# jeongminpark417/COALA-GNN

Hardware: AMD Instinct MI355X
Metric: feature-gather GB/s (payload = rows x dim x 4 B delivered per second), IGB-medium GraphSAGE minibatch fetch (higher is better)
Workload: dtype f32

## Files before the change

coala-gnn_amd/csrc/coala_cache.hip:

```cpp
#include <hip/hip_runtime.h>
#include <hip/hip_ext.h>

#include <algorithm>
#include <cstdarg>
#include <cstdio>
#include <cstdlib>
#include <cstring>
#include <new>
#include <type_traits>
#include <utility>
#include <vector>

#include "../../include/coala_hip.h"
#include "coala_internal.h"

namespace {

constexpr uint64_t kEmptyKey = 0xFFFFFFFFFFFFFFFFull;
constexpr uint32_t kLinkMiss = 0x80000000u;
constexpr uint32_t kLinkBad = 0x7FFFFFFFu;
constexpr int kStatBlocks = 2048;
constexpr int kFillSlots = 8;

struct CacheDev {
    void* keys;
    uint64_t* set_cnt;
    uint32_t* color_meta;
    int32_t* color_counters;
    const int32_t* node_color;
    float* lines;
    const float* cold;
    uint64_t num_sets;
    uint64_t num_rows;
    uint32_t cache_dim;
    uint32_t dim;
    uint32_t n_gpus;
    int32_t gshift;
    int32_t sshift;
    uint32_t distributed;
    uint32_t cold_partitioned;
    uint32_t tag32;
    uint64_t* set_head;
    uint32_t* miss_link;
    unsigned long long* stats;
};

__device__ __forceinline__ uint64_t set_of(const CacheDev& c, uint64_t id) {
    uint64_t k = id;
    if (c.distributed) {
        if (c.gshift >= 0) k = id >> c.gshift;
        else if ((id >> 32) == 0) k = (uint32_t)id / c.n_gpus;
        else k = id / c.n_gpus;
    }
    if (c.sshift >= 0) return k & (c.num_sets - 1);
    if ((k >> 32) == 0 && (c.num_sets >> 32) == 0) return (uint32_t)k % (uint32_t)c.num_sets;
    return k % c.num_sets;
}

__device__ __forceinline__ uint64_t cold_row_of(const CacheDev& c, uint64_t id) {
    if (!c.cold_partitioned) return id;
    if (c.gshift >= 0) return id >> c.gshift;
    return id / c.n_gpus;
}

constexpr int kMaxRanges = 64;
struct RangeSet {
// ... 62 lines not shown

constexpr int kK1MinWaves = 4;
constexpr int kK1Passes = 4;
constexpr int64_t kK1SingleMaxChunks = 1 << 20;
constexpr int kK1Waves = 2;
#ifdef COALA_DEV_KNOBS
constexpr int kK1MaxWaves = 4;
#else
constexpr int kK1MaxWaves = kK1Waves;
#endif

template <typename V> __device__ __forceinline__ V nt_load(const V* p) { return __builtin_nontemporal_load(p); }
template <typename V> __device__ __forceinline__ void nt_store(V v, V* p) { __builtin_nontemporal_store(v, p); }

template <int CD, int VEC, typename TAG, int NP, bool FULL, bool REDIR, bool SINGLE>
__global__ __launch_bounds__(64 * kK1MaxWaves, kK1MinWaves) void probe_gather_kernel(const int64_t* __restrict__ idx, float* __restrict__ out,
                                                                    int64_t n, uint32_t gen, uint32_t n_blocks, CacheDev c, Redirect rd) {
    using G = Geo<CD, VEC, NP>;
    using V = typename VecT<VEC>::type;
    using TG = TagGeo<TAG>;
    using TV = typename TG::vec;
    constexpr int R = G::R;
    static_assert(R <= 32, "per-chunk row masks are 32 bits wide");
    if (blockIdx.x == 0 && threadIdx.x < kFillSlots) reinterpret_cast<uint32_t*>(c.stats + 2 * kStatBlocks)[(gen & 1u) * kFillSlots + threadIdx.x] = 0u;
    uint32_t* fill_flag = reinterpret_cast<uint32_t*>(c.stats + 2 * kStatBlocks) + 2 * kFillSlots;
    if (blockIdx.x == 0 && threadIdx.x == kFillSlots) fill_flag[(gen + 1u) & 1u] = 0u;
    constexpr int TSTEPS = (R + TG::SPL - 1) / TG::SPL;
    int lane = threadIdx.x & 63;
#ifdef COALA_DEV_KNOBS
    const int wpb = (int)(blockDim.x >> 6);
#else
    constexpr int wpb = kK1Waves;
#endif
    const int64_t wave = (int64_t)blockIdx.x * wpb + (threadIdx.x >> 6);
    const int64_t n_waves = (int64_t)n_blocks * wpb;
    const int64_t n_chunks = (n + R - 1) / R;
    const uint32_t nunits = c.dim / VEC;
    const TAG* __restrict__ keys = reinterpret_cast<const TAG*>(c.keys);

    struct Ids { uint64_t id[TSTEPS]; bool valid[TSTEPS]; int32_t drow[REDIR ? TSTEPS : 1]; };
    struct Tags { uint64_t id[TSTEPS]; uint32_t set[TSTEPS]; TV kk[TSTEPS]; bool ok[TSTEPS]; bool valid[TSTEPS]; int32_t drow[REDIR ? TSTEPS : 1]; };
    auto load_ids = [&](int64_t chunk) {
        Ids r;
#pragma unroll
        for (int t = 0; t < TSTEPS; ++t) {
            const int q_l = t * TG::SPL + lane / TG::LPS;
            const int64_t i_l = chunk * R + q_l;
// ... 110 lines not shown
            }
#pragma unroll
            for (int v = 0; v < G::VPL; ++v) {
                const uint32_t u = v * G::LPR + l_in;
                if (FULL || u < nunits) {
                    if (h) dst[u] = val[p][v];
                    else if (bad) dst[u] = V(0.0f);
                }
            }
        }
#pragma unroll
        for (int t = 0; t < TSTEPS; ++t) {
            if (lead_l[t]) {
                uint32_t w = 0u;
                if (imiss_l[t]) w = kLinkMiss | (((uint32_t)(prev[t] >> 32) == gen) ? (uint32_t)prev[t] : 0u);
                else if (bad_l[t]) w = kLinkBad;
                c.miss_link[base + t * TG::SPL + lane / TG::LPS] = w;
            }
        }
        if (SINGLE) break;
    }
}

__device__ __forceinline__ uint64_t shfl64(uint64_t v, int src) {
    const uint32_t lo = __shfl((int)(uint32_t)v, src), hi = __shfl((int)(uint32_t)(v >> 32), src);
    return ((uint64_t)hi << 32) | lo;
}

template <int CD, int VEC, bool REDIR = false, int NP = 4>
__global__ __launch_bounds__(256) void miss_fill_kernel(CacheDev c, const int64_t* __restrict__ idx, float* __restrict__ out,
                                                        int tile_rows, int sparse_max, uint32_t gen, RangeSet rs, Redirect rd, int dyn_slot) {
    using G = Geo<CD, VEC, NP>;
    using V = typename VecT<VEC>::type;
    constexpr int R = G::R;
    const int lane = threadIdx.x & 63;
    const int64_t wave = (int64_t)blockIdx.x * (blockDim.x >> 6) + (threadIdx.x >> 6);
    const int64_t n_waves = (int64_t)gridDim.x * (blockDim.x >> 6);
    const int64_t n_tiles = ((int64_t)rs.total + tile_rows - 1) / tile_rows;
    const int chunks_per_tile = tile_rows / R;
    const uint32_t nunits = c.dim / VEC;
    const int sub = (G::RPP == 2) ? (lane >> 5) : 0;
    const int l_in = lane & (G::LPR - 1);
    uint32_t my_miss = 0, my_bad = 0;

    constexpr int U = 8;
    uint32_t* ticket = reinterpret_cast<uint32_t*>(c.stats + 2 * kStatBlocks) + (dyn_slot < 0 ? 0 : dyn_slot);
    const bool dyn = dyn_slot >= 0;
    if (reinterpret_cast<const uint32_t*>(c.stats + 2 * kStatBlocks)[2 * kFillSlots + (gen & 1u)] == 0u) return;
    const int64_t n_deal = dyn ? 1 : n_waves;
    const int64_t even8 = n_tiles / (n_waves * 8);
    const int claim_min = even8 < 1 ? 1 : (even8 > U ? U : (int)even8);
    int claim = claim_min;
    for (int64_t unit = dyn ? -1 : wave;;) {
      int64_t claim_end = n_tiles;
      if (dyn) {
          uint32_t t = 0;
          if (lane == 0) t = atomicAdd(ticket, (uint32_t)claim);
          unit = (int64_t)(uint32_t)__builtin_amdgcn_readfirstlane((int)t);
          if (unit >= n_tiles) break;
          claim_end = unit + claim < n_tiles ? unit + claim : n_tiles;
          claim = claim * 2 > 4 * U ? 4 * U : claim * 2;
      } else if (unit >= n_tiles) break;
     for (int64_t tile0 = unit; tile0 < claim_end; tile0 += n_deal * U) {
      const int n_here = dyn ? (int)(claim_end - tile0 < U ? claim_end - tile0 : U) : U;
      uint64_t st_pack = 0;
#pragma unroll
      for (int u = 0; u < U; ++u) {
          const int64_t tile = tile0 + u * n_deal;
          const uint32_t p = (u < n_here && tile < n_tiles && lane < tile_rows) ? pos_of(rs, (uint32_t)(tile * tile_rows + lane)) : 0xFFFFFFFFu;
          const uint32_t w = (p != 0xFFFFFFFFu) ? c.miss_link[p] : 0u;
          const uint64_t v = (w == 0u) ? 0u : ((w & kLinkMiss) ? 1u : 2u);
          st_pack |= v << (8 * u);
      }
      if (!__ballot(st_pack != 0)) continue;
      uint32_t slot_l = 0, win_l = 0;
      uint64_t id_l = 0;
      int64_t drow_l = 0;
      auto rank_at = [&](uint32_t pos) {
          id_l = (uint64_t)idx[pos];
          drow_l = (int64_t)pos;
          if (REDIR && (int64_t)pos >= rd.begin && (int64_t)pos < rd.end)
              drow_l = -((rd.row_map ? rd.row_map[(int64_t)pos - rd.begin] : (int64_t)pos - rd.begin) + 1);
          const uint64_t set = set_of(c, id_l);
          uint32_t cur = (uint32_t)c.set_head[set];
          uint32_t total = 0, rank = 0;
          while (cur) {
              const uint32_t p2 = cur - 1;
              ++total;
              rank += (p2 < pos) ? 1u : 0u;
              cur = c.miss_link[p2] & ~kLinkMiss;
          }
          const uint64_t cv = __hip_atomic_load(c.set_cnt + set, __ATOMIC_RELAXED, __HIP_MEMORY_SCOPE_AGENT);
          const uint32_t cnt0 = ((uint32_t)(cv >> 32) == gen) ? (uint32_t)cv - total : (uint32_t)cv;
          if (rank == 0) __hip_atomic_store(c.set_cnt + set, ((uint64_t)gen << 32) | (uint32_t)(cnt0 + total), __ATOMIC_RELAXED, __HIP_MEMORY_SCOPE_AGENT);
          const uint32_t way = (cnt0 + rank) & (COALA_WAYS - 1);
          slot_l = (uint32_t)(set * COALA_WAYS) + way;
          win_l = (rank + COALA_WAYS >= total) ? 1u : 0u;
          if (win_l) {
              if (c.tag32) reinterpret_cast<uint32_t*>(c.keys)[slot_l] = (uint32_t)id_l;
              else reinterpret_cast<uint64_t*>(c.keys)[slot_l] = id_l;
              if (c.color_counters) {
                  const int32_t col = c.node_color[id_l];
                  atomicSub(c.color_counters + c.color_meta[slot_l], 1);
                  atomicAdd(c.color_counters + col, 1);
                  c.color_meta[slot_l] = (uint32_t)col;
              }
          }
      };
      auto move_group = [&](const int (&srcl)[G::PASSES], const bool (&live)[G::PASSES]) {
          V val[G::PASSES][G::VPL];
          uint32_t slot_[G::PASSES];
          uint64_t id[G::PASSES];
          int64_t drow[G::PASSES];
          bool winner[G::PASSES];
#pragma unroll
          for (int p = 0; p < G::PASSES; ++p) {
              slot_[p] = (uint32_t)__shfl((int)slot_l, srcl[p]);
              winner[p] = __shfl((int)win_l, srcl[p]) != 0;
              id[p] = shfl64(id_l, srcl[p]);
              drow[p] = (int64_t)shfl64((uint64_t)drow_l, srcl[p]);
          }
#pragma unroll
          for (int p = 0; p < G::PASSES; ++p) {
              const V* src = reinterpret_cast<const V*>(c.cold + cold_row_of(c, id[p]) * (uint64_t)c.dim);
#pragma unroll
              for (int v = 0; v < G::VPL; ++v) {
                  const uint32_t u = v * G::LPR + l_in;
                  if (live[p] && u < nunits) val[p][v] = nt_load(src + u);
              }
          }
#pragma unroll
          for (int p = 0; p < G::PASSES; ++p) {
              V* dst = (REDIR && drow[p] < 0) ? reinterpret_cast<V*>(rd.out + (uint64_t)(-(drow[p] + 1)) * c.dim)
                                              : reinterpret_cast<V*>(out + (uint64_t)drow[p] * c.dim);
              V* line = reinterpret_cast<V*>(c.lines + (uint64_t)slot_[p] * CD);
#pragma unroll
              for (int v = 0; v < G::VPL; ++v) {
                  const uint32_t u = v * G::LPR + l_in;
                  if (live[p] && u < nunits) {
                      nt_store(val[p][v], dst + u);
                      if (winner[p]) nt_store(val[p][v], line + u);
                  }
              }
          }
      };
      auto stream_holders = [&](uint64_t holders) {
          int srcl[G::PASSES];
          bool live[G::PASSES];
          while (holders) {
#pragma unroll
              for (int p = 0; p < G::PASSES; ++p) {
                  int l0 = -1, l1 = -1;
                  if (holders) { l0 = __builtin_ctzll(holders); holders &= holders - 1; }
                  if (G::RPP == 2 && holders) { l1 = __builtin_ctzll(holders); holders &= holders - 1; }
                  const int l = (G::RPP == 2 && sub) ? l1 : l0;
                  live[p] = l >= 0;
                  srcl[p] = l >= 0 ? l : 0;
              }
              move_group(srcl, live);
          }
      };
      uint64_t mmask[U];
      uint32_t total_miss = 0, worst = 0;
#pragma unroll
      for (int u = 0; u < U; ++u) {
          const uint8_t st = (uint8_t)(st_pack >> (8 * u));
          mmask[u] = __ballot(st == 1);
          my_miss += (st == 1);
          my_bad += (st == 2);
          const uint32_t cnt = (uint32_t)__builtin_popcountll(mmask[u]);
          total_miss += cnt;
          worst = cnt > worst ? cnt : worst;
      }
      if (!total_miss) continue;
      claim = claim_min;
      if (total_miss <= 64 && (int)worst <= sparse_max) {
          uint32_t k = (uint32_t)lane;
          int u_sel = -1;
          uint64_t m_sel = 0;
#pragma unroll
          for (int u = 0; u < U; ++u) {
              const uint32_t cnt = (uint32_t)__builtin_popcountll(mmask[u]);
              if (u_sel < 0) {
                  if (k < cnt) { u_sel = u; m_sel = mmask[u]; }
                  else k -= cnt;
              }
          }
          if (u_sel >= 0) {
              for (uint32_t i = 0; i < k; ++i) m_sel &= m_sel - 1;
              const uint32_t pos = pos_of(rs, (uint32_t)((tile0 + u_sel * n_deal) * tile_rows + __builtin_ctzll(m_sel)));
              rank_at(pos);
          }
          stream_holders(total_miss >= 64 ? ~0ull : ((1ull << total_miss) - 1ull));
          continue;
      }
#pragma nounroll
      for (int u = 0; u < U; ++u) {
        const uint8_t st = (uint8_t)(st_pack >> (8 * u));
        const uint64_t tile_mask = __ballot(st == 1);
        if (!tile_mask) continue;
        const uint32_t pos_l = st ? pos_of(rs, (uint32_t)((tile0 + u * n_deal) * tile_rows + lane)) : 0u;
        if (__builtin_popcountll(tile_mask) <= sparse_max) {
            if (st == 1) rank_at(pos_l);
            stream_holders(tile_mask);
        } else {
            int srcl[G::PASSES];
            bool live[G::PASSES];
            for (int ck = 0; ck < chunks_per_tile; ++ck) {
                const uint32_t live_mask = (uint32_t)(tile_mask >> (ck * R)) & ((1u << R) - 1u);
                if (!live_mask) continue;
                const int lane0 = ck * R;
                if (st == 1 && lane >= lane0 && lane < lane0 + R) rank_at(pos_l);
#pragma unroll
                for (int p = 0; p < G::PASSES; ++p) {
                    const int q = p * G::RPP + sub;
                    live[p] = (live_mask >> q) & 1;
                    srcl[p] = lane0 + q;
                }
                move_group(srcl, live);
            }
        }
      }
     }
      if (!dyn) break;
    }
    __shared__ uint32_t s_m[256 / 64], s_b[256 / 64];
    for (int off = 32; off > 0; off >>= 1) { my_miss += __shfl_down(my_miss, off); my_bad += __shfl_down(my_bad, off); }
    if (lane == 0) { s_m[threadIdx.x >> 6] = my_miss; s_b[threadIdx.x >> 6] = my_bad; }
    __syncthreads();
    if (threadIdx.x == 0) {
        uint32_t m = 0, b = 0;
        for (int w = 0; w < (int)(blockDim.x >> 6); ++w) { m += s_m[w]; b += s_b[w]; }
        if (m) c.stats[2 * blockIdx.x] += m;
        if (b) c.stats[2 * blockIdx.x + 1] += b;
    }
}

template <int CD, int VEC, int NP = 4>
__global__ __launch_bounds__(256) void scatter_rows_kernel(float* __restrict__ out, const float* __restrict__ src,
                                                           const int64_t* __restrict__ map, RangeSet rs, uint32_t dim) {
    using G = Geo<CD, VEC, NP>;
    using V = typename VecT<VEC>::type;
    constexpr int R = G::R;
    const int lane = threadIdx.x & 63;
    const int64_t wave = (int64_t)blockIdx.x * (blockDim.x >> 6) + (threadIdx.x >> 6);
    const int64_t n_waves = (int64_t)gridDim.x * (blockDim.x >> 6);
    const int64_t n_chunks = ((int64_t)rs.total + R - 1) / R;
    const uint32_t nunits = dim / VEC;
    const int sub = (G::RPP == 2) ? (lane >> 5) : 0;
    const int l_in = lane & (G::LPR - 1);
    for (int64_t chunk = wave; chunk < n_chunks; chunk += n_waves) {
        const int64_t base = chunk * R;
        V val[G::PASSES][G::VPL];
        int64_t d[G::PASSES];
#pragma unroll
        for (int p = 0; p < G::PASSES; ++p) {
            const int64_t vr = base + p * G::RPP + sub;
// ... 99 lines not shown
            const uint64_t mask = __ballot(o == g);
            const int64_t bg = __shfl(off, (int)g);
            if (o == g) dest = bg + __builtin_popcountll(mask & ((1ull << lane) - 1ull));
            if ((uint32_t)lane == g) off += __builtin_popcountll(mask);
        }
        if (valid) {
            node_out[dest] = id;
            map_out[dest] = i;
        }
    }
}

}


namespace {

struct LaunchShape {
    int k1_grid_cap;
    int k1_waves;
    bool k1_single;
    int k1_passes;
    int k2_grid_cap;
    int k2_tile_rows;
    int k2_sparse_max;
    int k2_unit_tiles;
};

LaunchShape launch_shape(uint32_t cache_dim, bool host_tier) {
    LaunchShape s;
    s.k1_grid_cap = 16384;
    s.k1_waves = kK1Waves;
    s.k1_single = cache_dim >= 256;
    s.k1_passes = 0;
    const int host_blocks = std::min(64, std::max(24, 16 * 1024 / (int)cache_dim));
    s.k2_grid_cap = host_tier ? host_blocks : kStatBlocks;
    s.k2_tile_rows = host_tier ? 64 : 0;
    s.k2_sparse_max = host_tier ? 32 : 0;
    s.k2_unit_tiles = host_tier ? 1 : 0;
    return s;
}

#ifdef COALA_DEV_KNOBS
void apply_dev_knobs(LaunchShape& s) {
    if (const char* e = getenv("COALA_K1_PASSES")) { int v = atoi(e); if (v == 2 || v == 4 || v == 8 || v == 16) s.k1_passes = v; }
    if (const char* e = getenv("COALA_K1_GRID")) { int g = atoi(e); if (g >= 1 && g <= 65535) s.k1_grid_cap = g; }
    if (const char* e = getenv("COALA_K1_WAVES")) { int w = atoi(e); if (w == 1 || w == 2 || w == 4) s.k1_waves = w; }
    if (const char* e = getenv("COALA_K1_SINGLE")) s.k1_single = atoi(e) != 0;
    if (const char* e = getenv("COALA_K2_TILE_ROWS")) { int t = atoi(e); if (t == 0 || t == 8 || t == 16 || t == 32 || t == 64) s.k2_tile_rows = t; }
    if (const char* e = getenv("COALA_K2_GRID")) { int g = atoi(e); if (g >= 1 && g <= kStatBlocks) s.k2_grid_cap = g; }
    if (const char* e = getenv("COALA_K2_SPARSE")) { int g = atoi(e); if (g >= 0 && g <= 64) s.k2_sparse_max = g; }
    if (const char* e = getenv("COALA_K2_UNIT_TILES")) { int g = atoi(e); if (g >= 0 && g <= 1) s.k2_unit_tiles = g; }
}
#endif

}

struct coala_cache {
    coala_cache_config_t cfg;
    CacheDev d;
    uint64_t cap = 0;
    uint32_t gen = 0;
    int32_t* node_color_dev = nullptr;
    uint32_t* wave_counts = nullptr;
    uint64_t wave_counts_cap = 0;
    int64_t* route_bases = nullptr;
    struct EvPair { hipEvent_t a, b; int kind; uint64_t rows; };
    std::vector<EvPair> ev_live;
    std::vector<hipEvent_t> ev_pool;
    coala_cache_profile_t prof{};
    hipStream_t last_stream = nullptr;
    hipStream_t order_stream = nullptr;
    bool order_set = false;
    hipEvent_t order_ev = nullptr;
    uint64_t table_bytes = 0;
    LaunchShape shape;
    int32_t* color_pin = nullptr;
    int32_t* color_pin_async = nullptr;
    hipEvent_t color_ev = nullptr;
    int32_t color_pending = -1;
    int64_t open_batch_rows = -1;
    std::vector<std::pair<int64_t, int64_t>> open_filled;
    int64_t open_filled_rows = 0;
    Redirect open_redirect{0, 0, nullptr, nullptr};
    int fill_launches = 0;
    uint64_t rows_total = 0;
    uint64_t cum_hit = 0, cum_miss = 0;
    uint64_t prof_hit0 = 0, prof_miss0 = 0;
    bool fetch_events = false;
    static constexpr int kFetchRing = 2048;
    std::vector<hipEvent_t> fev;
    uint64_t fev_calls = 0;
    hipEvent_t last_begin = nullptr, last_end = nullptr;
};

namespace {

#define fail coala_fail_
#define HIPCHK COALA_HIPCHK

int follow_stream(coala_cache* h, hipStream_t s) {
    if (h->order_set && h->order_stream != s) {
        if (!h->order_ev) HIPCHK(hipEventCreateWithFlags(&h->order_ev, hipEventDisableTiming));
        if (hipEventRecord(h->order_ev, h->order_stream) == hipSuccess) HIPCHK(hipStreamWaitEvent(s, h->order_ev, 0));
        else (void)hipGetLastError();
    }
    h->order_stream = s;
    h->order_set = true;
    return COALA_OK;
}

int ilog2_exact(uint64_t v) {
    if (v == 0 || (v & (v - 1))) return -1;
    int s = 0;
    while ((1ull << s) != v) ++s;
    return s;
}

int ensure_scratch(coala_cache* h, uint64_t n, hipStream_t s) {
    if (n <= h->cap) return COALA_OK;
    HIPCHK(hipStreamSynchronize(s));
    uint64_t cap = h->cap ? h->cap : 1024;
    while (cap < n) cap *= 2;
    if (h->d.miss_link) HIPCHK(hipFree(h->d.miss_link));
    h->d.miss_link = nullptr;
    HIPCHK(hipMalloc((void**)&h->d.miss_link, cap * sizeof(uint32_t)));
    h->cap = cap;
    return COALA_OK;
}

hipEvent_t take_event(coala_cache* h) {
    if (!h->ev_pool.empty()) {
        hipEvent_t e = h->ev_pool.back();
        h->ev_pool.pop_back();
        return e;
    }
    hipEvent_t e = nullptr;
    if (hipEventCreate(&e) != hipSuccess) return nullptr;
    return e;
}

void drain_events(coala_cache* h) {
    for (auto& p : h->ev_live) {
        float ms = 0.f;
        if (hipEventSynchronize(p.b) == hipSuccess && hipEventElapsedTime(&ms, p.a, p.b) == hipSuccess) {
            if (p.kind == 0) { h->prof.gather_ms += ms; h->prof.gather_launches++; h->prof.gather_rows += p.rows; }
            else { h->prof.fill_ms += ms; h->prof.fill_launches++; }
        }
        h->ev_pool.push_back(p.a);
        h->ev_pool.push_back(p.b);
    }
    h->ev_live.clear();
}

struct ProfScope {
    coala_cache* h; hipStream_t s; int kind; uint64_t rows; hipEvent_t a = nullptr, b = nullptr; bool on;
    hipEvent_t xa = nullptr, xb = nullptr;
    ProfScope(coala_cache* h_, hipStream_t s_, int kind_, uint64_t rows_, hipEvent_t xa_ = nullptr, hipEvent_t xb_ = nullptr)
        : h(h_), s(s_), kind(kind_), rows(rows_), xa(xa_), xb(xb_) {
        on = (h->cfg.flags & COALA_FLAG_PROFILE) != 0;
        if (on) {
            if (h->ev_live.size() >= 8192) drain_events(h);
            a = take_event(h); b = take_event(h);
            on = a && b;
            if (on) h->last_stream = s;
        }
    }
    template <typename K, typename... Args>
    void launch(K kernel, dim3 grid, dim3 block, Args... args) {
        if (on) hipExtLaunchKernelGGL(kernel, grid, block, 0, s, a, b, 0, args...);
        else if (xa || xb) hipExtLaunchKernelGGL(kernel, grid, block, 0, s, xa, xb, 0, args...);
        else hipLaunchKernelGGL(kernel, grid, block, 0, s, args...);
    }
    ~ProfScope() {
        if (on) h->ev_live.push_back({a, b, kind, rows});
    }
};

template <typename F>
int dispatch_geo(uint32_t cache_dim, bool vec4, F&& f) {
    switch (cache_dim) {
        case 128: return vec4 ? f(Geo<128, 4>{}) : f(Geo<128, 1>{});
        case 256: return vec4 ? f(Geo<256, 4>{}) : f(Geo<256, 1>{});
        case 512: return vec4 ? f(Geo<512, 4>{}) : f(Geo<512, 1>{});
        case 1024: return vec4 ? f(Geo<1024, 4>{}) : f(Geo<1024, 1>{});
    }
    return fail(COALA_EINVAL, "unsupported cache_dim %u", cache_dim);
}

template <int CD, int VEC> constexpr int geo_cd(Geo<CD, VEC>) { return CD; }
template <int CD, int VEC> constexpr int geo_vec(Geo<CD, VEC>) { return VEC; }

inline bool aligned16(const void* p) { return (reinterpret_cast<uintptr_t>(p) & 15u) == 0; }

template <typename F>
int for_each_range_set(const int64_t* begins, const int64_t* ends, int count, F&& f) {
// ... 64 lines not shown
    d.num_rows = cfg->num_rows;
    d.cache_dim = (uint32_t)cd;
    d.dim = (uint32_t)cfg->dim;
    d.n_gpus = (uint32_t)cfg->n_gpus;
    d.gshift = ilog2_exact((uint64_t)cfg->n_gpus);
    d.sshift = ilog2_exact(sets);
    d.distributed = (cfg->flags & COALA_FLAG_DISTRIBUTED) ? 1u : 0u;
    d.cold_partitioned = (cfg->flags & COALA_FLAG_COLD_PARTITIONED) ? 1u : 0u;
    d.cold = cfg->cold_table;
    d.tag32 = (!(cfg->flags & COALA_FLAG_TAG64) && cfg->num_rows <= 0xFFFFFFFFull) ? 1u : 0u;
    const uint64_t tag_bytes = d.tag32 ? 4 : 8;
    int rc = COALA_OK;
    auto alloc = [&](void** p, uint64_t bytes) -> int {
        hipError_t e = hipMalloc(p, bytes);
        if (e != hipSuccess) return fail(COALA_ENOMEM, "hipMalloc(%llu) failed: %s", (unsigned long long)bytes, hipGetErrorString(e));
        h->table_bytes += bytes;
        return COALA_OK;
    };
    do {
        if ((rc = alloc((void**)&d.keys, slots * tag_bytes))) break;
        if ((rc = alloc((void**)&d.set_cnt, sets * 8))) break;
        if ((rc = alloc((void**)&d.color_meta, slots * 4))) break;
        if ((rc = alloc((void**)&d.set_head, sets * 8))) break;
        if ((rc = alloc((void**)&d.stats, (kStatBlocks * 2 + kFillSlots + 1) * 8))) break;
        if ((rc = alloc((void**)&d.lines, slots * (uint64_t)cd * 4))) break;
        if ((rc = alloc((void**)&h->route_bases, 65 * 8))) break;
        if (hipMemset(d.keys, 0xFF, slots * tag_bytes) != hipSuccess || hipMemset(d.set_cnt, 0, sets * 8) != hipSuccess ||
            hipMemset(d.color_meta, 0, slots * 4) != hipSuccess || hipMemset(d.set_head, 0, sets * 8) != hipSuccess ||
            hipMemset(d.stats, 0, (kStatBlocks * 2 + kFillSlots + 1) * 8) != hipSuccess) {
            rc = fail(COALA_EHIP, "hipMemset failed");
            break;
        }
        if (cfg->node_color) {
            if ((rc = alloc((void**)&d.color_counters, ((uint64_t)cfg->num_colors + 1) * 4))) break;
            if (hipMemset(d.color_counters, 0, ((uint64_t)cfg->num_colors + 1) * 4) != hipSuccess) { rc = fail(COALA_EHIP, "hipMemset failed"); break; }
            if ((rc = alloc((void**)&h->node_color_dev, cfg->num_rows * 4))) break;
            const uint64_t chunk = 1ull << 22;
            std::vector<int32_t> tmp((size_t)(cfg->num_rows < chunk ? cfg->num_rows : chunk));
            for (uint64_t off = 0; off < cfg->num_rows && rc == COALA_OK; off += chunk) {
                const uint64_t cnt = cfg->num_rows - off < chunk ? cfg->num_rows - off : chunk;
                for (uint64_t k = 0; k < cnt; ++k) {
                    const int64_t col = cfg->node_color[off + k];
                    if (col < 0 || col > cfg->num_colors) { rc = fail(COALA_EINVAL, "node_color[%llu]=%lld outside [0,%d]", (unsigned long long)(off + k), (long long)col, cfg->num_colors); break; }
                    tmp[k] = (int32_t)col;
                }
                if (rc == COALA_OK && hipMemcpy(h->node_color_dev + off, tmp.data(), cnt * 4, hipMemcpyHostToDevice) != hipSuccess)
                    rc = fail(COALA_EHIP, "colour upload failed");
            }
            if (rc) break;
            d.node_color = h->node_color_dev;
        }
        h->gen = 0;
// ... 7 lines not shown
#endif
        }
        if (cfg->max_batch) rc = ensure_scratch(h, cfg->max_batch, nullptr);
    } while (0);
    if (rc == COALA_OK && hipDeviceSynchronize() != hipSuccess) rc = fail(COALA_EHIP, "device sync failed after create");
    if (rc != COALA_OK) {
        coala_cache_destroy(h);
        return rc;
    }
    *out = h;
    return COALA_OK;
}

int coala_cache_destroy(coala_cache_t* h) {
    if (!h) return COALA_OK;
    (void)hipSetDevice(h->cfg.device);
    (void)hipDeviceSynchronize();
    drain_events(h);
    for (auto e : h->ev_pool) (void)hipEventDestroy(e);
    for (auto e : h->fev)
        if (e) (void)hipEventDestroy(e);
    CacheDev& d = h->d;
    void* ptrs[] = {d.keys, d.set_cnt, d.color_meta, d.set_head, d.stats, d.lines, d.color_counters,
                    h->node_color_dev, d.miss_link,
                    h->wave_counts, h->route_bases};
    for (void* p : ptrs)
        if (p) (void)hipFree(p);
    if (h->color_pin) (void)hipHostFree(h->color_pin);
    if (h->color_pin_async) (void)hipHostFree(h->color_pin_async);
    if (h->color_ev) (void)hipEventDestroy(h->color_ev);
    if (h->order_ev) (void)hipEventDestroy(h->order_ev);
    delete h;
    return COALA_OK;
}

int64_t coala_cache_row_dim(const coala_cache_t* h) { return h ? (int64_t)h->d.dim : 0; }

int coala_cache_fetch_events(coala_cache_t* h, int enable) {
    if (!h) return fail(COALA_EINVAL, "null handle");
    h->fetch_events = enable != 0;
    if (!h->fetch_events) h->last_begin = h->last_end = nullptr;
    return COALA_OK;
}

int coala_cache_last_fetch_events(const coala_cache_t* h, void** begin_ev, void** end_ev) {
    if (!h) return fail(COALA_EINVAL, "null handle");
    if (begin_ev) *begin_ev = (void*)h->last_begin;
// ... 73 lines not shown
            if (begins[k] < 0 || begins[k] > ends[k] || ends[k] > n)
                return fail(COALA_EINVAL, "fill range [%lld, %lld) outside the batch of %lld rows", (long long)begins[k], (long long)ends[k], (long long)n);
            if (ends[k] > begins[k]) add.emplace_back(begins[k], ends[k]);
        }
        if (phases == kPhaseFill) {
            std::vector<std::pair<int64_t, int64_t>> all = h->open_filled;
            all.insert(all.end(), add.begin(), add.end());
            std::sort(all.begin(), all.end());
            for (size_t k = 1; k < all.size(); ++k)
                if (all[k].first < all[k - 1].second)
                    return fail(COALA_EINVAL, "fill range [%lld, %lld) overlaps positions that were already filled in this batch", (long long)all[k].first, (long long)all[k].second);
            h->open_filled.swap(all);
        }
        for (auto& r : add) fill_rows += r.second - r.first;
        if (fill_rows == 0 && !(phases & kPhaseProbe)) return COALA_OK;
    }
    hipStream_t s = (hipStream_t)stream;
    HIPCHK(hipSetDevice(h->cfg.device));
    if (int rc_ = follow_stream(h, s)) return rc_;
    int rc = ensure_scratch(h, (uint64_t)n, s);
    if (rc) return rc;
    if (phases & kPhaseProbe) {
        h->fill_launches = 0;
        if (++h->gen == 0) {
            HIPCHK(hipMemsetAsync(h->d.set_head, 0, h->d.num_sets * 8, s));
            HIPCHK(hipMemset2DAsync(reinterpret_cast<char*>(h->d.set_cnt) + 4, 8, 0, 4, h->d.num_sets, s));
            h->gen = 1;
        }
        if (!(phases & kPhaseFill)) {
            h->open_batch_rows = n;
            h->open_filled.clear();
            h->open_filled_rows = 0;
            h->open_redirect = rd;
        }
    }
    const uint32_t gen = h->gen;
    const bool redir = rd.end > rd.begin;
    const bool vec4 = (h->d.dim % 4 == 0) && aligned16(out) && aligned16(h->d.cold) && (!redir || aligned16(rd.out));
    CacheDev d = h->d;
    if (force_dist) d.distributed = 1u;
    hipEvent_t fe_begin = nullptr, fe_end = nullptr;
    if (h->fetch_events && phases == kPhaseBoth && !(h->cfg.flags & COALA_FLAG_PROFILE)) {
        if (h->fev.empty()) h->fev.assign(2 * (size_t)coala_cache::kFetchRing, nullptr);
        const size_t slot = (size_t)(h->fev_calls % coala_cache::kFetchRing);
        for (size_t k = 2 * slot; k < 2 * slot + 2; ++k)
            if (!h->fev[k]) HIPCHK(hipEventCreate(&h->fev[k]));
// ... 33 lines not shown
                    constexpr bool S = decltype(single_c)::value;
                    if (redir) return full ? probe_gather_kernel<CD, VEC, TAG, NPR, true, true, S> : probe_gather_kernel<CD, VEC, TAG, NPR, false, true, S>;
                    return full ? probe_gather_kernel<CD, VEC, TAG, NP, true, false, S> : probe_gather_kernel<CD, VEC, TAG, NP, false, false, S>;
                };
                ps.launch(single ? pick(std::true_type{}) : pick(std::false_type{}), grid, block, idx, out, n, gen, (uint32_t)grid.x, d, rd);
            };
#ifdef COALA_DEV_KNOBS
            if (h->shape.k1_passes) {
                auto by_np = [&](auto tag_c) {
                    switch (h->shape.k1_passes) {
                        case 2: launch_k1(tag_c, std::integral_constant<int, 2>{}); break;
                        case 8: launch_k1(tag_c, std::integral_constant<int, 8>{}); break;
                        case 16: launch_k1(tag_c, std::integral_constant<int, (Geo<CD, VEC, 16>::R <= 32 ? 16 : 8)>{}); break;
                        default: launch_k1(tag_c, std::integral_constant<int, 4>{}); break;
                    }
                };
                if (d.tag32) by_np(uint32_t{}); else by_np(uint64_t{});
            } else
#endif
            if (d.tag32) launch_k1(uint32_t{}, std::integral_constant<int, kK1Passes>{});
            else launch_k1(uint64_t{}, std::integral_constant<int, kK1Passes>{});
        }
        if ((phases & kPhaseFill) && fill_rows > 0) {
            const int tile_rows = h->shape.k2_tile_rows > 0 ? h->shape.k2_tile_rows : G::R;
            return for_each_range_set(begins, ends, n_ranges, [&](const RangeSet& rs) -> int {
                const bool last_set = ++set_no == n_sets;
                ProfScope ps(h, s, 2, 0, nullptr, last_set ? fe_end : nullptr);
                if (rode && last_set) rode[1] = ps.on ? ps.b : fe_end;
                const int64_t tiles = ((int64_t)rs.total + tile_rows - 1) / tile_rows;
                const dim3 grid(grid_for(tiles, 4, h->shape.k2_grid_cap));
                const int64_t waves = (int64_t)grid.x * 4;
                int dyn_slot = -1;
                if (h->shape.k2_unit_tiles > 0 && tiles > waves && tiles < 0x7FFFFFFF && h->fill_launches < kFillSlots)
                    dyn_slot = (int)((gen & 1u) * kFillSlots) + h->fill_launches;
                h->fill_launches++;
                if (redir) ps.launch(miss_fill_kernel<CD, VEC, true>, grid, dim3(256), d, idx, out, tile_rows, h->shape.k2_sparse_max, gen, rs, rd, dyn_slot);
                else ps.launch(miss_fill_kernel<CD, VEC, false>, grid, dim3(256), d, idx, out, tile_rows, h->shape.k2_sparse_max, gen, rs, rd, dyn_slot);
                return COALA_OK;
            });
        }
        return COALA_OK;
    });
    if (rc) return rc;
    if (own_ring) {
        h->last_begin = fe_begin;
        h->last_end = fe_end;
        h->fev_calls++;
    }
    if (phases & kPhaseProbe) h->rows_total += (uint64_t)n;
    if (phases == kPhaseFill) {
        h->open_filled_rows += fill_rows;
        if (h->open_filled_rows == h->open_batch_rows) {
            h->open_batch_rows = -1;
            h->open_filled.clear();
            h->open_filled_rows = 0;
        }
    }
    HIPCHK(hipGetLastError());
    if (h->cfg.flags & COALA_FLAG_SYNC) HIPCHK(hipStreamSynchronize(s));
    return COALA_OK;
// ... 251 lines not shown
```

Baseline: 81.65.

## Split miss fill into rank kernel that compacts a miss list and streaming copy kernel

Replaces the single miss_fill_kernel, which ranked misses and streamed cold rows in the same wave with tile/sparse heuristics, with two kernels. The first ranks each miss, updates tags and colour counters, and appends a compact record (cold row, winner flag, destination row, cache slot) to a device list through a wave-level atomic. The second streams cold rows densely from that list into the output and cache lines, with optional dynamic ticket claiming. This removes divergence and sparse-tile inefficiency in the copy phase. It costs an extra launch, a list write and read, and extra scratch memory.

Measured after the change: 81.74 (median of 6 runs). No clear change (+0.1%).

```diff
diff --git a/coala-gnn_amd/csrc/coala_cache.hip b/coala-gnn_amd/csrc/coala_cache.hip
--- a/coala-gnn_amd/csrc/coala_cache.hip
+++ b/coala-gnn_amd/csrc/coala_cache.hip
@@ -42,6 +42,7 @@
     uint32_t tag32;
     uint64_t* set_head;
     uint32_t* miss_link;
+    void* fill_list;
     unsigned long long* stats;
 };
 
@@ -150,7 +151,11 @@
     using TV = typename TG::vec;
     constexpr int R = G::R;
     static_assert(R <= 32, "per-chunk row masks are 32 bits wide");
-    if (blockIdx.x == 0 && threadIdx.x < kFillSlots) reinterpret_cast<uint32_t*>(c.stats + 2 * kStatBlocks)[(gen & 1u) * kFillSlots + threadIdx.x] = 0u;
+    if (blockIdx.x == 0 && threadIdx.x < kFillSlots) {
+        uint32_t* ctl = reinterpret_cast<uint32_t*>(c.stats + 2 * kStatBlocks);
+        ctl[(gen & 1u) * kFillSlots + threadIdx.x] = 0u;
+        ctl[2 * kFillSlots + 2 + (gen & 1u) * kFillSlots + threadIdx.x] = 0u;
+    }
     uint32_t* fill_flag = reinterpret_cast<uint32_t*>(c.stats + 2 * kStatBlocks) + 2 * kFillSlots;
     if (blockIdx.x == 0 && threadIdx.x == kFillSlots) fill_flag[(gen + 1u) & 1u] = 0u;
     constexpr int TSTEPS = (R + TG::SPL - 1) / TG::SPL;
@@ -307,207 +312,68 @@
     }
 }
 
-__device__ __forceinline__ uint64_t shfl64(uint64_t v, int src) {
-    const uint32_t lo = __shfl((int)(uint32_t)v, src), hi = __shfl((int)(uint32_t)(v >> 32), src);
-    return ((uint64_t)hi << 32) | lo;
-}
-
-template <int CD, int VEC, bool REDIR = false, int NP = 4>
-__global__ __launch_bounds__(256) void miss_fill_kernel(CacheDev c, const int64_t* __restrict__ idx, float* __restrict__ out,
-                                                        int tile_rows, int sparse_max, uint32_t gen, RangeSet rs, Redirect rd, int dyn_slot) {
-    using G = Geo<CD, VEC, NP>;
-    using V = typename VecT<VEC>::type;
-    constexpr int R = G::R;
+constexpr int kCtlFlag = 2 * kFillSlots, kCtlCount = 2 * kFillSlots + 2, kCtlSpare = 4 * kFillSlots + 2, kCtlWords = 4 * kFillSlots + 4;
+__device__ __forceinline__ uint32_t* ctl_words(const CacheDev& c) { return reinterpret_cast<uint32_t*>(c.stats + 2 * kStatBlocks); }
+
+typedef vu32x4 FillRec;
+constexpr uint32_t kRecWinner = 0x80000000u;
+
+__global__ __launch_bounds__(256) void miss_rank_kernel(CacheDev c, const int64_t* __restrict__ idx, uint32_t gen, RangeSet rs, Redirect rd,
+                                                        FillRec* __restrict__ list, uint32_t* __restrict__ count, uint32_t room) {
+    if (ctl_words(c)[kCtlFlag + (gen & 1u)] == 0u) return;
     const int lane = threadIdx.x & 63;
     const int64_t wave = (int64_t)blockIdx.x * (blockDim.x >> 6) + (threadIdx.x >> 6);
     const int64_t n_waves = (int64_t)gridDim.x * (blockDim.x >> 6);
-    const int64_t n_tiles = ((int64_t)rs.total + tile_rows - 1) / tile_rows;
-    const int chunks_per_tile = tile_rows / R;
-    const uint32_t nunits = c.dim / VEC;
-    const int sub = (G::RPP == 2) ? (lane >> 5) : 0;
-    const int l_in = lane & (G::LPR - 1);
+    const int64_t n_tiles = ((int64_t)rs.total + 63) / 64;
     uint32_t my_miss = 0, my_bad = 0;
-
-    constexpr int U = 8;
-    uint32_t* ticket = reinterpret_cast<uint32_t*>(c.stats + 2 * kStatBlocks) + (dyn_slot < 0 ? 0 : dyn_slot);
-    const bool dyn = dyn_slot >= 0;
-    if (reinterpret_cast<const uint32_t*>(c.stats + 2 * kStatBlocks)[2 * kFillSlots + (gen & 1u)] == 0u) return;
-    const int64_t n_deal = dyn ? 1 : n_waves;
-    const int64_t even8 = n_tiles / (n_waves * 8);
-    const int claim_min = even8 < 1 ? 1 : (even8 > U ? U : (int)even8);
-    int claim = claim_min;
-    for (int64_t unit = dyn ? -1 : wave;;) {
-      int64_t claim_end = n_tiles;
-      if (dyn) {
-          uint32_t t = 0;
-          if (lane == 0) t = atomicAdd(ticket, (uint32_t)claim);
-          unit = (int64_t)(uint32_t)__builtin_amdgcn_readfirstlane((int)t);
-          if (unit >= n_tiles) break;
-          claim_end = unit + claim < n_tiles ? unit + claim : n_tiles;
-          claim = claim * 2 > 4 * U ? 4 * U : claim * 2;
-      } else if (unit >= n_tiles) break;
-     for (int64_t tile0 = unit; tile0 < claim_end; tile0 += n_deal * U) {
-      const int n_here = dyn ? (int)(claim_end - tile0 < U ? claim_end - tile0 : U) : U;
-      uint64_t st_pack = 0;
-#pragma unroll
-      for (int u = 0; u < U; ++u) {
-          const int64_t tile = tile0 + u * n_deal;
-          const uint32_t p = (u < n_here && tile < n_tiles && lane < tile_rows) ? pos_of(rs, (uint32_t)(tile * tile_rows + lane)) : 0xFFFFFFFFu;
-          const uint32_t w = (p != 0xFFFFFFFFu) ? c.miss_link[p] : 0u;
-          const uint64_t v = (w == 0u) ? 0u : ((w & kLinkMiss) ? 1u : 2u);
-          st_pack |= v << (8 * u);
-      }
-      if (!__ballot(st_pack != 0)) continue;
-      uint32_t slot_l = 0, win_l = 0;
-      uint64_t id_l = 0;
-      int64_t drow_l = 0;
-      auto rank_at = [&](uint32_t pos) {
-          id_l = (uint64_t)idx[pos];
-          drow_l = (int64_t)pos;
-          if (REDIR && (int64_t)pos >= rd.begin && (int64_t)pos < rd.end)
-              drow_l = -((rd.row_map ? rd.row_map[(int64_t)pos - rd.begin] : (int64_t)pos - rd.begin) + 1);
-          const uint64_t set = set_of(c, id_l);
-          uint32_t cur = (uint32_t)c.set_head[set];
-          uint32_t total = 0, rank = 0;
-          while (cur) {
-              const uint32_t p2 = cur - 1;
-              ++total;
-              rank += (p2 < pos) ? 1u : 0u;
-              cur = c.miss_link[p2] & ~kLinkMiss;
-          }
-          const uint64_t cv = __hip_atomic_load(c.set_cnt + set, __ATOMIC_RELAXED, __HIP_MEMORY_SCOPE_AGENT);
-          const uint32_t cnt0 = ((uint32_t)(cv >> 32) == gen) ? (uint32_t)cv - total : (uint32_t)cv;
-          if (rank == 0) __hip_atomic_store(c.set_cnt + set, ((uint64_t)gen << 32) | (uint32_t)(cnt0 + total), __ATOMIC_RELAXED, __HIP_MEMORY_SCOPE_AGENT);
-          const uint32_t way = (cnt0 + rank) & (COALA_WAYS - 1);
-          slot_l = (uint32_t)(set * COALA_WAYS) + way;
-          win_l = (rank + COALA_WAYS >= total) ? 1u : 0u;
-          if (win_l) {
-              if (c.tag32) reinterpret_cast<uint32_t*>(c.keys)[slot_l] = (uint32_t)id_l;
-              else reinterpret_cast<uint64_t*>(c.keys)[slot_l] = id_l;
-              if (c.color_counters) {
-                  const int32_t col = c.node_color[id_l];
-                  atomicSub(c.color_counters + c.color_meta[slot_l], 1);
-                  atomicAdd(c.color_counters + col, 1);
-                  c.color_meta[slot_l] = (uint32_t)col;
-              }
-          }
-      };
-      auto move_group = [&](const int (&srcl)[G::PASSES], const bool (&live)[G::PASSES]) {
-          V val[G::PASSES][G::VPL];
-          uint32_t slot_[G::PASSES];
-          uint64_t id[G::PASSES];
-          int64_t drow[G::PASSES];
-          bool winner[G::PASSES];
-#pragma unroll
-          for (int p = 0; p < G::PASSES; ++p) {
-              slot_[p] = (uint32_t)__shfl((int)slot_l, srcl[p]);
-              winner[p] = __shfl((int)win_l, srcl[p]) != 0;
-              id[p] = shfl64(id_l, srcl[p]);
-              drow[p] = (int64_t)shfl64((uint64_t)drow_l, srcl[p]);
-          }
-#pragma unroll
-          for (int p = 0; p < G::PASSES; ++p) {
-              const V* src = reinterpret_cast<const V*>(c.cold + cold_row_of(c, id[p]) * (uint64_t)c.dim);
-#pragma unroll
-              for (int v = 0; v < G::VPL; ++v) {
-                  const uint32_t u = v * G::LPR + l_in;
-                  if (live[p] && u < nunits) val[p][v] = nt_load(src + u);
-              }
-          }
-#pragma unroll
-          for (int p = 0; p < G::PASSES; ++p) {
-              V* dst = (REDIR && drow[p] < 0) ? reinterpret_cast<V*>(rd.out + (uint64_t)(-(drow[p] + 1)) * c.dim)
-                                              : reinterpret_cast<V*>(out + (uint64_t)drow[p] * c.dim);
-              V* line = reinterpret_cast<V*>(c.lines + (uint64_t)slot_[p] * CD);
-#pragma unroll
-              for (int v = 0; v < G::VPL; ++v) {
-                  const uint32_t u = v * G::LPR + l_in;
-                  if (live[p] && u < nunits) {
-                      nt_store(val[p][v], dst + u);
-                      if (winner[p]) nt_store(val[p][v], line + u);
-                  }
-              }
-          }
-      };
-      auto stream_holders = [&](uint64_t holders) {
-          int srcl[G::PASSES];
-          bool live[G::PASSES];
-          while (holders) {
-#pragma unroll
-              for (int p = 0; p < G::PASSES; ++p) {
-                  int l0 = -1, l1 = -1;
-                  if (holders) { l0 = __builtin_ctzll(holders); holders &= holders - 1; }
-                  if (G::RPP == 2 && holders) { l1 = __builtin_ctzll(holders); holders &= holders - 1; }
-                  const int l = (G::RPP == 2 && sub) ? l1 : l0;
-                  live[p] = l >= 0;
-                  srcl[p] = l >= 0 ? l : 0;
-              }
-              move_group(srcl, live);
-          }
-      };
-      uint64_t mmask[U];
-      uint32_t total_miss = 0, worst = 0;
-#pragma unroll
-      for (int u = 0; u < U; ++u) {
-          const uint8_t st = (uint8_t)(st_pack >> (8 * u));
-          mmask[u] = __ballot(st == 1);
-          my_miss += (st == 1);
-          my_bad += (st == 2);
-          const uint32_t cnt = (uint32_t)__builtin_popcountll(mmask[u]);
-          total_miss += cnt;
-          worst = cnt > worst ? cnt : worst;
-      }
-      if (!total_miss) continue;
-      claim = claim_min;
-      if (total_miss <= 64 && (int)worst <= sparse_max) {
-          uint32_t k = (uint32_t)lane;
-          int u_sel = -1;
-          uint64_t m_sel = 0;
-#pragma unroll
-          for (int u = 0; u < U; ++u) {
-              const uint32_t cnt = (uint32_t)__builtin_popcountll(mmask[u]);
-              if (u_sel < 0) {
-                  if (k < cnt) { u_sel = u; m_sel = mmask[u]; }
-                  else k -= cnt;
-              }
-          }
-          if (u_sel >= 0) {
-              for (uint32_t i = 0; i < k; ++i) m_sel &= m_sel - 1;
-              const uint32_t pos = pos_of(rs, (uint32_t)((tile0 + u_sel * n_deal) * tile_rows + __builtin_ctzll(m_sel)));
-              rank_at(pos);
-          }
-          stream_holders(total_miss >= 64 ? ~0ull : ((1ull << total_miss) - 1ull));
-          continue;
-      }
-#pragma nounroll
-      for (int u = 0; u < U; ++u) {
-        const uint8_t st = (uint8_t)(st_pack >> (8 * u));
-        const uint64_t tile_mask = __ballot(st == 1);
-        if (!tile_mask) continue;
-        const uint32_t pos_l = st ? pos_of(rs, (uint32_t)((tile0 + u * n_deal) * tile_rows + lane)) : 0u;
-        if (__builtin_popcountll(tile_mask) <= sparse_max) {
-            if (st == 1) rank_at(pos_l);
-            stream_holders(tile_mask);
-        } else {
-            int srcl[G::PASSES];
-            bool live[G::PASSES];
-            for (int ck = 0; ck < chunks_per_tile; ++ck) {
-                const uint32_t live_mask = (uint32_t)(tile_mask >> (ck * R)) & ((1u << R) - 1u);
-                if (!live_mask) continue;
-                const int lane0 = ck * R;
-                if (st == 1 && lane >= lane0 && lane < lane0 + R) rank_at(pos_l);
-#pragma unroll
-                for (int p = 0; p < G::PASSES; ++p) {
-                    const int q = p * G::RPP + sub;
-                    live[p] = (live_mask >> q) & 1;
-                    srcl[p] = lane0 + q;
+    for (int64_t tile = wave; tile < n_tiles; tile += n_waves) {
+        const int64_t v = tile * 64 + lane;
+        const uint32_t pos = v < (int64_t)rs.total ? pos_of(rs, (uint32_t)v) : 0xFFFFFFFFu;
+        const uint32_t w = (pos != 0xFFFFFFFFu) ? c.miss_link[pos] : 0u;
+        const bool miss = (w & kLinkMiss) != 0u;
+        my_miss += miss;
+        my_bad += (w == kLinkBad);
+        const uint64_t mask = __ballot(miss);
+        if (!mask) continue;
+        FillRec rec = FillRec(0u);
+        if (miss) {
+            const uint64_t id = (uint64_t)idx[pos];
+            int64_t drow = (int64_t)pos;
+            if ((int64_t)pos >= rd.begin && (int64_t)pos < rd.end)
+                drow = -((rd.row_map ? rd.row_map[(int64_t)pos - rd.begin] : (int64_t)pos - rd.begin) + 1);
+            const uint64_t set = set_of(c, id);
+            uint32_t cur = (uint32_t)c.set_head[set];
+            uint32_t total = 0, rank = 0;
+            while (cur) {
+                const uint32_t p2 = cur - 1;
+                ++total;
+                rank += (p2 < pos) ? 1u : 0u;
+                cur = c.miss_link[p2] & ~kLinkMiss;
+            }
+            const uint64_t cv = __hip_atomic_load(c.set_cnt + set, __ATOMIC_RELAXED, __HIP_MEMORY_SCOPE_AGENT);
+            const uint32_t cnt0 = ((uint32_t)(cv >> 32) == gen) ? (uint32_t)cv - total : (uint32_t)cv;
+            if (rank == 0) __hip_atomic_store(c.set_cnt + set, ((uint64_t)gen << 32) | (uint32_t)(cnt0 + total), __ATOMIC_RELAXED, __HIP_MEMORY_SCOPE_AGENT);
+            const uint32_t way = (cnt0 + rank) & (COALA_WAYS - 1);
+            const uint32_t slot = (uint32_t)(set * COALA_WAYS) + way;
+            const bool win = rank + COALA_WAYS >= total;
+            if (win) {
+                if (c.tag32) reinterpret_cast<uint32_t*>(c.keys)[slot] = (uint32_t)id;
+                else reinterpret_cast<uint64_t*>(c.keys)[slot] = id;
+                if (c.color_counters) {
+                    const int32_t col = c.node_color[id];
+                    atomicSub(c.color_counters + c.color_meta[slot], 1);
+                    atomicAdd(c.color_counters + col, 1);
+                    c.color_meta[slot] = (uint32_t)col;
                 }
-                move_group(srcl, live);
             }
-        }
-      }
-     }
-      if (!dyn) break;
+            const uint64_t crow = cold_row_of(c, id);
+            rec = FillRec{(uint32_t)crow, (uint32_t)(crow >> 32) | (win ? kRecWinner : 0u), (uint32_t)(int32_t)drow, slot};
+        }
+        uint32_t base = 0;
+        if (lane == 0) base = atomicAdd(count, (uint32_t)__builtin_popcountll(mask));
+        base = (uint32_t)__builtin_amdgcn_readfirstlane((int)base);
+        const uint32_t at = base + (uint32_t)__builtin_popcountll(mask & ((1ull << lane) - 1ull));
+        if (miss && at < room) list[at] = rec;
     }
     __shared__ uint32_t s_m[256 / 64], s_b[256 / 64];
     for (int off = 32; off > 0; off >>= 1) { my_miss += __shfl_down(my_miss, off); my_bad += __shfl_down(my_bad, off); }
@@ -518,6 +384,82 @@
         for (int w = 0; w < (int)(blockDim.x >> 6); ++w) { m += s_m[w]; b += s_b[w]; }
         if (m) c.stats[2 * blockIdx.x] += m;
         if (b) c.stats[2 * blockIdx.x + 1] += b;
+    }
+}
+
+template <int CD, int VEC, int NP = 4>
+__global__ __launch_bounds__(256) void miss_stream_kernel(CacheDev c, float* __restrict__ out, float* __restrict__ rd_out, uint32_t gen,
+                                                          const FillRec* __restrict__ list, const uint32_t* __restrict__ count,
+                                                          uint32_t room, uint32_t* __restrict__ ticket, uint32_t claim) {
+    using G = Geo<CD, VEC, NP>;
+    using V = typename VecT<VEC>::type;
+    constexpr int R = G::R;
+    if (ctl_words(c)[kCtlFlag + (gen & 1u)] == 0u) return;
+    const int lane = threadIdx.x & 63;
+    const uint32_t wave = blockIdx.x * (blockDim.x >> 6) + (threadIdx.x >> 6);
+    const uint32_t n_waves = gridDim.x * (blockDim.x >> 6);
+    const uint32_t n_rec = *count < room ? *count : room;
+    const uint32_t n_groups = (n_rec + R - 1) / R;
+    const uint32_t nunits = c.dim / VEC;
+    const int sub = (G::RPP == 2) ? (lane >> 5) : 0;
+    const int l_in = lane & (G::LPR - 1);
+    V val[G::PASSES][G::VPL];
+    FillRec rec[G::PASSES];
+    bool live[G::PASSES];
+    auto load_group = [&](uint32_t g) {
+#pragma unroll
+        for (int p = 0; p < G::PASSES; ++p) {
+            const uint32_t r = g * R + p * G::RPP + sub;
+            live[p] = r < n_rec;
+            rec[p] = live[p] ? list[r] : FillRec(0u);
+        }
+#pragma unroll
+        for (int p = 0; p < G::PASSES; ++p) {
+            const uint64_t crow = ((uint64_t)(rec[p].y & ~kRecWinner) << 32) | rec[p].x;
+            const V* src = reinterpret_cast<const V*>(c.cold + crow * (uint64_t)c.dim);
+#pragma unroll
+            for (int v = 0; v < G::VPL; ++v) {
+                const uint32_t u = v * G::LPR + l_in;
+                if (live[p] && u < nunits) val[p][v] = nt_load(src + u);
+            }
+        }
+    };
+    auto store_group = [&]() {
+#pragma unroll
+        for (int p = 0; p < G::PASSES; ++p) {
+            const int32_t drow = (int32_t)rec[p].z;
+            const bool winner = (rec[p].y & kRecWinner) != 0u;
+            V* dst = drow < 0 ? reinterpret_cast<V*>(rd_out + (uint64_t)(-((int64_t)drow + 1)) * c.dim)
+                              : reinterpret_cast<V*>(out + (uint64_t)drow * c.dim);
+            V* line = reinterpret_cast<V*>(c.lines + (uint64_t)rec[p].w * CD);
+#pragma unroll
+            for (int v = 0; v < G::VPL; ++v) {
+                const uint32_t u = v * G::LPR + l_in;
+                if (live[p] && u < nunits) {
+                    nt_store(val[p][v], dst + u);
+                    if (winner) nt_store(val[p][v], line + u);
+                }
+            }
+        }
+    };
+    if (!ticket) {
+        for (uint32_t g = wave; g < n_groups; g += n_waves) { load_group(g); store_group(); }
+        return;
+    }
+    auto draw = [&]() {
+        uint32_t t = 0;
+        if (lane == 0) t = atomicAdd(ticket, claim);
+        return (uint32_t)__builtin_amdgcn_readfirstlane((int)t);
+    };
+    for (uint32_t g0 = draw(); g0 < n_groups;) {
+        const uint32_t g1 = g0 + claim < n_groups ? g0 + claim : n_groups;
+        uint32_t next = 0;
+        for (uint32_t g = g0; g < g1; ++g) {
+            load_group(g);
+            if (g + 1 == g1) next = draw();
+            store_group();
+        }
+        g0 = next;
     }
 }
 
@@ -663,9 +605,8 @@
     bool k1_single;
     int k1_passes;
     int k2_grid_cap;
-    int k2_tile_rows;
-    int k2_sparse_max;
-    int k2_unit_tiles;
+    int k2_claim_rows;
+    bool k2_dynamic;
 };
 
 LaunchShape launch_shape(uint32_t cache_dim, bool host_tier) {
@@ -676,9 +617,8 @@
     s.k1_passes = 0;
     const int host_blocks = std::min(64, std::max(24, 16 * 1024 / (int)cache_dim));
     s.k2_grid_cap = host_tier ? host_blocks : kStatBlocks;
-    s.k2_tile_rows = host_tier ? 64 : 0;
-    s.k2_sparse_max = host_tier ? 32 : 0;
-    s.k2_unit_tiles = host_tier ? 1 : 0;
+    s.k2_claim_rows = 0;
+    s.k2_dynamic = host_tier;
     return s;
 }
 
@@ -688,10 +628,9 @@
     if (const char* e = getenv("COALA_K1_GRID")) { int g = atoi(e); if (g >= 1 && g <= 65535) s.k1_grid_cap = g; }
     if (const char* e = getenv("COALA_K1_WAVES")) { int w = atoi(e); if (w == 1 || w == 2 || w == 4) s.k1_waves = w; }
     if (const char* e = getenv("COALA_K1_SINGLE")) s.k1_single = atoi(e) != 0;
-    if (const char* e = getenv("COALA_K2_TILE_ROWS")) { int t = atoi(e); if (t == 0 || t == 8 || t == 16 || t == 32 || t == 64) s.k2_tile_rows = t; }
+    if (const char* e = getenv("COALA_K2_TILE_ROWS")) { int t = atoi(e); if (t == 0 || t == 8 || t == 16 || t == 32 || t == 64) s.k2_claim_rows = t; }
     if (const char* e = getenv("COALA_K2_GRID")) { int g = atoi(e); if (g >= 1 && g <= kStatBlocks) s.k2_grid_cap = g; }
-    if (const char* e = getenv("COALA_K2_SPARSE")) { int g = atoi(e); if (g >= 0 && g <= 64) s.k2_sparse_max = g; }
-    if (const char* e = getenv("COALA_K2_UNIT_TILES")) { int g = atoi(e); if (g >= 0 && g <= 1) s.k2_unit_tiles = g; }
+    if (const char* e = getenv("COALA_K2_UNIT_TILES")) { int g = atoi(e); if (g >= 0 && g <= 1) s.k2_dynamic = g != 0; }
 }
 #endif
 
@@ -725,6 +664,7 @@
     int64_t open_filled_rows = 0;
     Redirect open_redirect{0, 0, nullptr, nullptr};
     int fill_launches = 0;
+    int64_t fill_rows_dealt = 0;
     uint64_t rows_total = 0;
     uint64_t cum_hit = 0, cum_miss = 0;
     uint64_t prof_hit0 = 0, prof_miss0 = 0;
@@ -764,8 +704,12 @@
     uint64_t cap = h->cap ? h->cap : 1024;
     while (cap < n) cap *= 2;
     if (h->d.miss_link) HIPCHK(hipFree(h->d.miss_link));
+    if (h->d.fill_list) HIPCHK(hipFree(h->d.fill_list));
     h->d.miss_link = nullptr;
+    h->d.fill_list = nullptr;
+    h->cap = 0;
     HIPCHK(hipMalloc((void**)&h->d.miss_link, cap * sizeof(uint32_t)));
+    HIPCHK(hipMalloc(&h->d.fill_list, 2 * cap * sizeof(FillRec)));
     h->cap = cap;
     return COALA_OK;
 }
@@ -808,11 +752,13 @@
         }
     }
     template <typename K, typename... Args>
-    void launch(K kernel, dim3 grid, dim3 block, Args... args) {
-        if (on) hipExtLaunchKernelGGL(kernel, grid, block, 0, s, a, b, 0, args...);
-        else if (xa || xb) hipExtLaunchKernelGGL(kernel, grid, block, 0, s, xa, xb, 0, args...);
+    void launch_part(bool first, bool last, K kernel, dim3 grid, dim3 block, Args... args) {
+        const hipEvent_t ea = first ? (on ? a : xa) : nullptr, eb = last ? (on ? b : xb) : nullptr;
+        if (ea || eb) hipExtLaunchKernelGGL(kernel, grid, block, 0, s, ea, eb, 0, args...);
         else hipLaunchKernelGGL(kernel, grid, block, 0, s, args...);
     }
+    template <typename K, typename... Args>
+    void launch(K kernel, dim3 grid, dim3 block, Args... args) { launch_part(true, true, kernel, grid, block, args...); }
     ~ProfScope() {
         if (on) h->ev_live.push_back({a, b, kind, rows});
     }
@@ -923,12 +869,12 @@
         if ((rc = alloc((void**)&d.set_cnt, sets * 8))) break;
         if ((rc = alloc((void**)&d.color_meta, slots * 4))) break;
         if ((rc = alloc((void**)&d.set_head, sets * 8))) break;
-        if ((rc = alloc((void**)&d.stats, (kStatBlocks * 2 + kFillSlots + 1) * 8))) break;
+        if ((rc = alloc((void**)&d.stats, kStatBlocks * 2 * 8 + kCtlWords * 4))) break;
         if ((rc = alloc((void**)&d.lines, slots * (uint64_t)cd * 4))) break;
         if ((rc = alloc((void**)&h->route_bases, 65 * 8))) break;
         if (hipMemset(d.keys, 0xFF, slots * tag_bytes) != hipSuccess || hipMemset(d.set_cnt, 0, sets * 8) != hipSuccess ||
             hipMemset(d.color_meta, 0, slots * 4) != hipSuccess || hipMemset(d.set_head, 0, sets * 8) != hipSuccess ||
-            hipMemset(d.stats, 0, (kStatBlocks * 2 + kFillSlots + 1) * 8) != hipSuccess) {
+            hipMemset(d.stats, 0, kStatBlocks * 2 * 8 + kCtlWords * 4) != hipSuccess) {
             rc = fail(COALA_EHIP, "hipMemset failed");
             break;
         }
@@ -982,7 +928,7 @@
         if (e) (void)hipEventDestroy(e);
     CacheDev& d = h->d;
     void* ptrs[] = {d.keys, d.set_cnt, d.color_meta, d.set_head, d.stats, d.lines, d.color_counters,
-                    h->node_color_dev, d.miss_link,
+                    h->node_color_dev, d.miss_link, d.fill_list,
                     h->wave_counts, h->route_bases};
     for (void* p : ptrs)
         if (p) (void)hipFree(p);
@@ -1102,6 +1048,7 @@
     if (rc) return rc;
     if (phases & kPhaseProbe) {
         h->fill_launches = 0;
+        h->fill_rows_dealt = 0;
         if (++h->gen == 0) {
             HIPCHK(hipMemsetAsync(h->d.set_head, 0, h->d.num_sets * 8, s));
             HIPCHK(hipMemset2DAsync(reinterpret_cast<char*>(h->d.set_cnt) + 4, 8, 0, 4, h->d.num_sets, s));
@@ -1181,20 +1128,30 @@
             else launch_k1(uint64_t{}, std::integral_constant<int, kK1Passes>{});
         }
         if ((phases & kPhaseFill) && fill_rows > 0) {
-            const int tile_rows = h->shape.k2_tile_rows > 0 ? h->shape.k2_tile_rows : G::R;
+            const uint32_t claim = (uint32_t)std::max(1, h->shape.k2_claim_rows / G::R);
+            uint32_t* ctl = reinterpret_cast<uint32_t*>(d.stats + 2 * kStatBlocks);
             return for_each_range_set(begins, ends, n_ranges, [&](const RangeSet& rs) -> int {
                 const bool last_set = ++set_no == n_sets;
                 ProfScope ps(h, s, 2, 0, nullptr, last_set ? fe_end : nullptr);
                 if (rode && last_set) rode[1] = ps.on ? ps.b : fe_end;
-                const int64_t tiles = ((int64_t)rs.total + tile_rows - 1) / tile_rows;
-                const dim3 grid(grid_for(tiles, 4, h->shape.k2_grid_cap));
-                const int64_t waves = (int64_t)grid.x * 4;
-                int dyn_slot = -1;
-                if (h->shape.k2_unit_tiles > 0 && tiles > waves && tiles < 0x7FFFFFFF && h->fill_launches < kFillSlots)
-                    dyn_slot = (int)((gen & 1u) * kFillSlots) + h->fill_launches;
+                uint32_t *count, *ticket;
+                if (h->fill_launches < kFillSlots) {
+                    const int slot = (int)((gen & 1u) * kFillSlots) + h->fill_launches;
+                    count = ctl + kCtlCount + slot;
+                    ticket = ctl + slot;
+                } else {
+                    count = ctl + kCtlSpare;
+                    ticket = ctl + kCtlSpare + 1;
+                    HIPCHK(hipMemsetAsync(count, 0, 8, s));
+                }
                 h->fill_launches++;
-                if (redir) ps.launch(miss_fill_kernel<CD, VEC, true>, grid, dim3(256), d, idx, out, tile_rows, h->shape.k2_sparse_max, gen, rs, rd, dyn_slot);
-                else ps.launch(miss_fill_kernel<CD, VEC, false>, grid, dim3(256), d, idx, out, tile_rows, h->shape.k2_sparse_max, gen, rs, rd, dyn_slot);
+                FillRec* list = reinterpret_cast<FillRec*>(d.fill_list) + (uint64_t)(gen & 1u) * h->cap + (uint64_t)h->fill_rows_dealt;
+                h->fill_rows_dealt += rs.total;
+                const dim3 rank_grid(grid_for(((int64_t)rs.total + 63) / 64, 4, kStatBlocks));
+                const dim3 grid(grid_for(((int64_t)rs.total + G::R - 1) / G::R, 4, h->shape.k2_grid_cap));
+                ps.launch_part(true, false, miss_rank_kernel, rank_grid, dim3(256), d, idx, gen, rs, rd, list, count, rs.total);
+                ps.launch_part(false, true, miss_stream_kernel<CD, VEC>, grid, dim3(256), d, out, redir ? rd.out : nullptr, gen, (const FillRec*)list, (const uint32_t*)count,
+                               rs.total, h->shape.k2_dynamic ? ticket : nullptr, claim);
                 return COALA_OK;
             });
         }
```
